# SciML/NonlinearSolve.jl

Hardware: AMD Instinct MI355X
Metric: newton_steps_per_sec (higher is better)
Workload: dtype f64; 1 GPU; bratu2d_1024x1024_newtonraphson_gmres30_fixedwork_csr_spmv; unknowns_global=1048576, unknowns_per_gpu=1048576, arnoldi_steps_per_newton_step=30, ortho=sstep_auto_auto, parallelism=row-range x1, comm=none

## Files before the change

include/mi355x_nk.h:

```cpp
#ifndef MI355X_NK_H
#define MI355X_NK_H

#include <stdint.h>
#include <stddef.h>

#ifdef __cplusplus
extern "C" {
#endif

#define NK_VERSION_MAJOR 0
#define NK_VERSION_MINOR 1

typedef enum {
  NK_OK = 0,
  NK_E_INVALID = -1,
  NK_E_HIP = -2,
  NK_E_RCCL = -3,
  NK_E_NOMEM = -4,
  NK_E_UNSUPPORTED = -5,
  NK_E_CALLBACK = -6,
  NK_E_SINGULAR = -7,
  NK_E_COMM = -8
} nk_status;

// ... 194 lines not shown
int nk_ctx_comm_init_callbacks(nk_ctx *ctx, int nranks, int rank, const nk_comm_callbacks *cb);
#define NK_IPC_HANDLE_BYTES 64
int nk_ctx_comm_peer_handle(nk_ctx *ctx, int64_t arena_bytes, char handle_out[NK_IPC_HANDLE_BYTES]);
int nk_ctx_comm_enable_peer(nk_ctx *ctx, const char *handles);
int nk_ctx_comm_peer_status(nk_ctx *ctx, int *enabled, int64_t *errors);
int nk_ctx_comm_allreduce(nk_ctx *ctx, double *buf, int count, int op);
int nk_ctx_comm_peer_selftest(nk_ctx *ctx, int *ok);
int nk_ctx_comm_peer_disable(nk_ctx *ctx);
int nk_ctx_comm_info(nk_ctx *ctx, int *kind, int *nranks, int *rank);
int nk_ctx_comm_device_shared(nk_ctx *ctx, int *shared);

int nk_partition_range(int64_t n_global, int64_t granule, int nranks, int rank,
                       int64_t *row_begin, int64_t *row_end);

int nk_csr_create(nk_ctx *ctx, int64_t nrows_local, int64_t n_global, int64_t row_begin, int64_t nnz,
                  int index_bits, int index_base, const void *rowptr, const void *colind,
                  const double *vals, int memspace, nk_csr **out);
int nk_csr_create_from_csc(nk_ctx *ctx, int64_t n, int64_t nnz, int index_bits, int index_base,
                           const void *colptr, const void *rowval, const double *nzval, nk_csr **out);
int nk_csr_create_from_csc_rows(nk_ctx *ctx, int64_t n, int64_t nnz, int index_bits, int index_base,
                                const void *colptr, const void *rowval, const double *nzval,
                                int64_t row_begin, int64_t nrows_local, nk_csr **out);
int nk_csr_destroy(nk_csr *A);
int nk_csr_set_values(nk_csr *A, const double *vals, int memspace);
int nk_csr_set_values_csc(nk_csr *A, const double *nzval, int64_t nnz_csc, int memspace);
int nk_csr_get_values(nk_csr *A, double *vals, int memspace);
int nk_csr_info(nk_csr *A, int64_t *nrows_local, int64_t *n_global, int64_t *nnz, int64_t *n_halo);
double *nk_csr_values_device(nk_csr *A);
int nk_spmv(nk_csr *A, const double *x, double *y, int memspace);
int nk_spmv_t(nk_csr *A, const double *x, double *y, int memspace);
int nk_csr_powers(nk_csr *A, const double *x, double *Y, int64_t ldy, int s, const double *theta, double scale, int memspace,
                  int *resident);
int nk_csr_powers_layout(int64_t nrows, const int32_t *rowptr, const int32_t *col, int num_cus, int layout[6]);
int nk_csr_colsumsq(nk_csr *A, double *out, int memspace);

int nk_problem_create(nk_ctx *ctx, int kind, const double *params, int nparams, nk_problem **out);
int nk_problem_create_user(nk_ctx *ctx, int64_t n_local, int64_t n_global, int64_t row_begin,
                           const nk_user_callbacks *cb, void *user, nk_csr *jac_pattern,
                           nk_problem **out);
int nk_problem_destroy(nk_problem *P);
int nk_problem_size(nk_problem *P, int64_t *n_local, int64_t *n_global, int64_t *row_begin);
int nk_problem_set_params(nk_problem *P, const double *params, int nparams);
int nk_problem_initial_guess(nk_problem *P, double *u0, int memspace);
int nk_residual(nk_problem *P, const double *u, double *f, int memspace);
int nk_jvp(nk_problem *P, const double *u, const double *v, double *Jv, int memspace);
int nk_vjp(nk_problem *P, const double *u, const double *v, double *vJ, int memspace);
int nk_problem_jac_csr(nk_problem *P, nk_csr **out);
int nk_jac_values(nk_problem *P, const double *u, int memspace, nk_csr *J);
int nk_jac_values_colored(nk_problem *P, const double *u, int memspace, nk_csr *J, int *ncolors);

int nk_gmres_create(nk_ctx *ctx, int64_t n_local, int restart_m, int ortho, nk_gmres **out);
int nk_gmres_destroy(nk_gmres *G);
int nk_gmres_set_operator_csr(nk_gmres *G, nk_csr *A);
int nk_gmres_set_operator_jvp(nk_gmres *G, nk_problem *P, const double *u, int memspace);
int nk_gmres_set_operator_fn(nk_gmres *G, nk_matvec_fn fn, void *user);
int nk_gmres_set_normal_form(nk_gmres *G, int on);
int nk_gmres_set_block_size(nk_gmres *G, int s);
int nk_gmres_set_sstep_basis(nk_gmres *G, int basis);
int nk_gmres_set_spectrum_interval(nk_gmres *G, double lo, double hi);
int nk_gmres_get_sstep_state(nk_gmres *G, int *block_size, int *newton_basis, int *breakdowns);
int nk_gmres_set_normal_form_damping(nk_gmres *G, const double *d_diag, double lambda);
int nk_gmres_set_shift(nk_gmres *G, double sigma);
int nk_gmres_set_shift_weights(nk_gmres *G, const double *d_m);
int nk_gmres_set_right_preconditioner(nk_gmres *G, nk_matvec_fn fn, void *user);
int nk_gmres_set_left_preconditioner(nk_gmres *G, nk_matvec_fn fn, void *user);
int nk_gmres_set_left_preconditioner_host(nk_gmres *G, nk_matvec_fn fn, void *user);
// ... 118 lines not shown
```

nonlinearsolve.jl_amd/_lib.py:

```python
from __future__ import annotations

import ctypes as C
import os
import subprocess

_HERE = os.path.dirname(os.path.abspath(__file__))
LIB_PATH = os.environ.get("NK_LIB_PATH") or os.path.join(_HERE, "lib", "libmi355x_nk.so")
CSRC = os.path.join(_HERE, "csrc")


class NKError(RuntimeError):
    pass


HOST, DEVICE = 0, 1
BATCH_ANALYTIC_JAC, BATCH_FLOAT32 = 1, 2
RET_NAMES = ["Default", "Success", "MaxIters", "Unstable", "Stalled", "InternalLinearSolveFailed",
             "ShrinkThresholdExceeded", "MaxTime", "Failure", "InternalLineSearchFailed"]
PROBLEM_QUADRATIC, PROBLEM_BRATU2D, PROBLEM_BRUSSELATOR2D, PROBLEM_USER = 1, 2, 3, 100
ALG_NEWTON_RAPHSON, ALG_TRUST_REGION, ALG_GAUSS_NEWTON, ALG_LEVENBERG_MARQUARDT, ALG_PSEUDO_TRANSIENT = 0, 1, 2, 3, 4
LINSOLVE_GMRES_MATFREE, LINSOLVE_GMRES_CSR, LINSOLVE_BANDED_LU = 0, 1, 2
ORTHO_MGS, ORTHO_CGS2, ORTHO_CGS, ORTHO_DCGS2, ORTHO_DCGS2_1R, ORTHO_SSTEP = 0, 1, 2, 3, 4, 5
FORCING_NONE, FORCING_EW2 = 0, 1
COMM_NONE, COMM_RCCL, COMM_CALLBACKS = 0, 1, 2
# ... 86 lines not shown
    "nk_ctx_synchronize": (_I, [_P]),
    "nk_ctx_set_halo_overlap": (_I, [_P, _I]),
    "nk_ctx_set_deterministic": (_I, [_P, _I]),
    "nk_ctx_profile_enable": (_I, [_P, _I]),
    "nk_ctx_profile_kernel_count": (_I, []),
    "nk_ctx_profile_query": (_I, [_P, _I, C.POINTER(C.c_char_p), C.POINTER(_L), C.POINTER(_D), C.POINTER(_D)]),
    "nk_comm_unique_id": (_I, [C.c_char_p]),
    "nk_ctx_comm_init_rccl": (_I, [_P, _I, _I, C.c_char_p]),
    "nk_ctx_comm_init_callbacks": (_I, [_P, _I, _I, C.POINTER(CommCallbacks)]),
    "nk_ctx_comm_info": (_I, [_P, C.POINTER(_I), C.POINTER(_I), C.POINTER(_I)]),
    "nk_ctx_comm_device_shared": (_I, [_P, C.POINTER(_I)]),
    "nk_ctx_comm_peer_handle": (_I, [_P, _L, C.c_char_p]),
    "nk_ctx_comm_enable_peer": (_I, [_P, C.c_char_p]),
    "nk_ctx_comm_peer_status": (_I, [_P, C.POINTER(_I), C.POINTER(_L)]),
    "nk_ctx_comm_peer_selftest": (_I, [_P, C.POINTER(_I)]),
    "nk_ctx_comm_peer_disable": (_I, [_P]),
    "nk_ctx_comm_allreduce": (_I, [_P, _P, _I, _I]),
    "nk_vec_axpby": (_I, [_P, _L, _D, _P, _D, _P]),
    "nk_vec_fill": (_I, [_P, _L, _D, _P]),
    "nk_partition_range": (_I, [_L, _L, _I, _I, C.POINTER(_L), C.POINTER(_L)]),
    "nk_csr_create": (_I, [_P, _L, _L, _L, _L, _I, _I, _P, _P, _P, _I, _PP]),
    "nk_csr_create_from_csc": (_I, [_P, _L, _L, _I, _I, _P, _P, _P, _PP]),
    "nk_csr_create_from_csc_rows": (_I, [_P, _L, _L, _I, _I, _P, _P, _P, _L, _L, _PP]),
    "nk_csr_destroy": (_I, [_P]),
    "nk_csr_set_values": (_I, [_P, _P, _I]),
    "nk_csr_get_values": (_I, [_P, _P, _I]),
    "nk_csr_set_values_csc": (_I, [_P, _P, _L, _I]),
    "nk_csr_info": (_I, [_P, C.POINTER(_L), C.POINTER(_L), C.POINTER(_L), C.POINTER(_L)]),
    "nk_csr_values_device": (_P, [_P]),
    "nk_spmv": (_I, [_P, _P, _P, _I]),
    "nk_spmv_t": (_I, [_P, _P, _P, _I]),
    "nk_csr_powers": (_I, [_P, _P, _P, _L, _I, _P, _D, _I, _P]),
    "nk_csr_powers_layout": (_I, [_L, _P, _P, _I, _P]),
    "nk_csr_colsumsq": (_I, [_P, _P, _I]),
    "nk_gmres_set_normal_form_damping": (_I, [_P, _P, C.c_double]),
    "nk_gmres_set_shift": (_I, [_P, C.c_double]),
    "nk_gmres_set_block_size": (_I, [_P, _I]),
    "nk_gmres_set_sstep_basis": (_I, [_P, _I]),
    "nk_gmres_set_spectrum_interval": (_I, [_P, C.c_double, C.c_double]),
    "nk_gmres_get_sstep_state": (_I, [_P, C.POINTER(_I), C.POINTER(_I), C.POINTER(_I)]),
    "nk_gmres_set_shift_weights": (_I, [_P, _P]),
    "nk_problem_create": (_I, [_P, _I, C.POINTER(_D), _I, _PP]),
    "nk_problem_create_user": (_I, [_P, _L, _L, _L, C.POINTER(UserCallbacks), _P, _P, _PP]),
    "nk_problem_destroy": (_I, [_P]),
    "nk_problem_size": (_I, [_P, C.POINTER(_L), C.POINTER(_L), C.POINTER(_L)]),
    "nk_problem_set_params": (_I, [_P, C.POINTER(_D), _I]),
    "nk_problem_initial_guess": (_I, [_P, _P, _I]),
    "nk_residual": (_I, [_P, _P, _P, _I]),
    "nk_jvp": (_I, [_P, _P, _P, _P, _I]),
    "nk_vjp": (_I, [_P, _P, _P, _P, _I]),
    "nk_problem_jac_csr": (_I, [_P, _PP]),
    "nk_jac_values": (_I, [_P, _P, _I, _P]),
    "nk_jac_values_colored": (_I, [_P, _P, _I, _P, C.POINTER(_I)]),
    "nk_gmres_create": (_I, [_P, _L, _I, _I, _PP]),
    "nk_gmres_destroy": (_I, [_P]),
    "nk_gmres_set_operator_csr": (_I, [_P, _P]),
    "nk_gmres_set_operator_jvp": (_I, [_P, _P, _P, _I]),
    "nk_gmres_set_operator_fn": (_I, [_P, MATVEC_FN, _P]),
    "nk_gmres_set_normal_form": (_I, [_P, _I]),
    "nk_gmres_set_right_preconditioner": (_I, [_P, MATVEC_FN, _P]),
    "nk_gmres_set_operator_fn_host": (_I, [_P, MATVEC_FN, _P]),
    "nk_gmres_set_right_preconditioner_host": (_I, [_P, MATVEC_FN, _P]),
    "nk_gmres_set_left_preconditioner": (_I, [_P, MATVEC_FN, _P]),
    "nk_gmres_set_left_preconditioner_host": (_I, [_P, MATVEC_FN, _P]),
    "nk_gmres_set_preconditioner": (_I, [_P, _I, _P]),
    "nk_precond_create_jacobi": (_I, [_P, _PP]),
# ... 98 lines not shown
```

nonlinearsolve.jl_amd/core.py:

```python
from __future__ import annotations

import ctypes as C
from dataclasses import dataclass, field
from typing import Callable, Optional, Sequence

import numpy as np

from . import _lib as L
from ._lib import NKError, check

try:
    import torch
except Exception:
    torch = None


def _is_torch(x):
    return torch is not None and isinstance(x, torch.Tensor)


def _ptr(x, n: Optional[int] = None):
    if _is_torch(x):
        if x.dtype != torch.float64:
            raise TypeError("device vectors must be float64")
# ... 252 lines not shown
        p, ms, _k = _ptr(vals, self.info()["nnz"])
        check(L.lib().nk_csr_set_values(self._h, p, ms))

    def values(self):
        out = np.empty(self.info()["nnz"])
        check(L.lib().nk_csr_get_values(self._h, C.c_void_p(out.ctypes.data), L.HOST))
        return out

    def values_device(self):
        return _view(L.lib().nk_csr_values_device(self._h), self.info()["nnz"])

    def matvec(self, x, out=None):
        n = self.info()["nrows_local"]
        px, ms, _k = _ptr(x, n)
        y = _like(x, n) if out is None else out
        py, ms2, _k2 = _ptr(y, n)
        if ms != ms2:
            raise ValueError("x and out must live in the same memory space")
        check(L.lib().nk_spmv(self._h, px, py, ms))
        return y

    def powers(self, x, s, theta=None, scale=1.0):
        n = self.info()["nrows_local"]
        px, ms, _k = _ptr(x, n)
        Y = _like(x, n * s)
        pY, _ms2, _k2 = _ptr(Y, n * s)
        th = None if theta is None else np.ascontiguousarray(theta, dtype=np.float64)
        if th is not None and th.size != s:
            raise ValueError("theta must have s entries")
        res = C.c_int(0)
        check(L.lib().nk_csr_powers(self._h, px, pY, n, int(s), None if th is None else C.c_void_p(th.ctypes.data),
                                    float(scale), ms, C.byref(res)))
        return Y.reshape(s, n), bool(res.value)

    @staticmethod
    def powers_layout(A, num_cus: int = 256):
        import numpy as _np
        A = A.tocsr()
        rp = _np.ascontiguousarray(A.indptr, dtype=_np.int32)
        ci = _np.ascontiguousarray(A.indices, dtype=_np.int32)
        out = (C.c_int * 6)()
        check(L.lib().nk_csr_powers_layout(int(A.shape[0]), C.c_void_p(rp.ctypes.data), C.c_void_p(ci.ctypes.data), int(num_cus), out))
        return {"kind": ("none", "bands", "segments")[out[0]], "slices": out[1], "slots": out[2], "bands": out[3],
                "segments": out[4], "ring": bool(out[5])}

    def rmatvec(self, x, out=None):
        n = self.info()["nrows_local"]
        px, ms, _k = _ptr(x, n)
        y = _like(x, n) if out is None else out
        py, _ms2, _k2 = _ptr(y, n)
        check(L.lib().nk_spmv_t(self._h, px, py, ms))
        return y

    def colsumsq(self, like=None):
        n = self.info()["nrows_local"]
        y = np.empty(n) if like is None else _like(like, n)
        py, ms, _k = _ptr(y, n)
        check(L.lib().nk_csr_colsumsq(self._h, py, ms))
        return y

    __matmul__ = matvec

    def close(self):
        if self._h and self._owned:
            L.lib().nk_csr_destroy(self._h)
        self._h = None
# ... 1209 lines not shown
```

nonlinearsolve.jl_amd/csrc/nk_powers.hip:

```cpp
#include <algorithm>
#include <stdlib.h>
#include <vector>

#include "nk_internal.h"

constexpr int PW_T = 1024;
constexpr int PW_HALO = 1024;
constexpr int PW_FLAG_STRIDE = 16;
constexpr int PW_NXCD = 8;

struct pw_args {
  int nrows, nb, s, variant;
  const int32_t *rowptr, *col;
  const double *val;
  const double *x0;
  double *Y;
  int64_t ldy;
  const double *scal_first, *scal_rest, *theta;
  const int *d_skip;
  uint64_t *flags;
  uint64_t base;
  uint64_t *err;
  int ns;
  double c_lap;
  const double *diag;
  int seg_len, ring;
  struct {
    int up, dn;
    const int32_t *halo_vl;
    double *push_up, *push_dn;
    uint64_t *flag_up, *flag_dn;
    const double *recv_up, *recv_dn;
    const uint64_t *myflag_up, *myflag_dn;
    uint64_t *err;
    int ebuf;
  } pr;
};

constexpr int PW_NST = 12, PW_STP = 16;
__device__ unsigned long long *g_pw_stamp = nullptr;
#ifdef NK_PW_STAMPS
#define PW_STAMP(p, i) do { if (t == 0 && (p) < PW_STP) s_pw_st[(p) * PW_NST + (i)] = wall_clock64(); } while (0)
#else
#define PW_STAMP(p, i) do { } while (0)
#endif

__device__ __forceinline__ int pw_band_of(int bid, int nb) {
  const int q = nb / PW_NXCD, r = nb % PW_NXCD;
  const int x = bid % PW_NXCD, k = bid / PW_NXCD;
  return x * q + (x < r ? x : r) + k;
}
__device__ __forceinline__ void pw_store_sc1(double *p, double v) {
  __hip_atomic_store(reinterpret_cast<unsigned long long *>(p), (unsigned long long)__double_as_longlong(v), __ATOMIC_RELAXED,
                     __HIP_MEMORY_SCOPE_AGENT);
}
// ... 15 lines not shown
      }
    }
  }
}
__device__ __forceinline__ bool pw_wait_peer(const uint64_t *f, uint64_t target, uint64_t *perr, uint64_t *err) {
  if (__hip_atomic_load(f, __ATOMIC_ACQUIRE, __HIP_MEMORY_SCOPE_SYSTEM) >= target) return true;
  const unsigned long long t0 = wall_clock64(), lim = nk_peer_timeout(perr);
  for (unsigned it = 1;; ++it) {
    __builtin_amdgcn_s_sleep(1);
    if (__hip_atomic_load(f, __ATOMIC_ACQUIRE, __HIP_MEMORY_SCOPE_SYSTEM) >= target) return true;
    if ((it & 63u) == 0) {
      if (__hip_atomic_load(err, __ATOMIC_RELAXED, __HIP_MEMORY_SCOPE_SYSTEM) != 0) return false;
      if (__hip_atomic_load(perr, __ATOMIC_RELAXED, __HIP_MEMORY_SCOPE_AGENT) > 4 || wall_clock64() - t0 > lim) {
        atomicAdd((unsigned long long *)perr, 1ull);
        __hip_atomic_store(err, (uint64_t)1, __ATOMIC_RELAXED, __HIP_MEMORY_SCOPE_SYSTEM);
        return false;
      }
    }
  }
}
__device__ __forceinline__ void pw_store_sys(double *p, double v) {
  __hip_atomic_store(reinterpret_cast<unsigned long long *>(p), (unsigned long long)__double_as_longlong(v), __ATOMIC_RELAXED,
                     __HIP_MEMORY_SCOPE_SYSTEM);
}
__device__ __forceinline__ double pw_load_sys(const double *p) {
  return __longlong_as_double((long long)__hip_atomic_load(reinterpret_cast<const unsigned long long *>(p), __ATOMIC_RELAXED,
                                                           __HIP_MEMORY_SCOPE_SYSTEM));
}
template <int RPT>
__device__ __forceinline__ constexpr int pw_slice(int q) {
  return q == 0 ? 0 : (q == 1 ? RPT - 1 : q - 1);
}

template <int RPT, int W, int GEN, bool PEER = false>
__global__ __launch_bounds__(PW_T) void k_spmv_powers(const pw_args a) {
  if (a.d_skip != nullptr && *a.d_skip != 0) return;
  extern __shared__ double pw_x[];
  __shared__ int s_abort;
#ifdef NK_PW_STAMPS
  __shared__ unsigned long long s_pw_st[PW_STP * PW_NST];
  for (int i = threadIdx.x; i < PW_STP * PW_NST; i += PW_T) s_pw_st[i] = 0;
#endif
  constexpr int RB = PW_T * RPT, XN = RB + 2 * PW_HALO;
  constexpr int NBND = RPT > 1 ? 2 : 1;
  const int t = threadIdx.x;
  const int b = pw_band_of(blockIdx.x, a.nb);
  const int r0 = b * RB;
  double *xa = pw_x, *xb = pw_x + XN;
  const bool pup = PEER && b == 0 && a.pr.up != 0, pdn = PEER && b == a.nb - 1 && a.pr.dn != 0;

  double v[RPT][W];
  int ci[RPT][W];
  int len[RPT];
  if constexpr (GEN == 1) {
    static_assert(W >= 5, "the 5-point stencil needs five slots per row");
#pragma unroll
    for (int i = 0; i < RPT; ++i) {
      const int r = r0 + t + PW_T * i;
      const int rc = r < a.nrows ? r : a.nrows - 1;
      const int gj = rc / a.ns, gi = rc - gj * a.ns;
      const double dd = a.diag[rc];
      const int base = rc - (r0 - PW_HALO), own = PW_HALO + t + PW_T * i;
      const bool hs = gj > 0, hw = gi > 0, he = gi + 1 < a.ns, hn = gj + 1 < a.ns;
      const int pW = hs ? 1 : 0, pC = pW + (hw ? 1 : 0), pE = pC + 1, pN = pE + (he ? 1 : 0), n = pN + (hn ? 1 : 0);
      const double off = -a.c_lap, ctr = 4.0 * a.c_lap - dd;
#pragma unroll
      for (int j = 0; j < W; ++j) {
        double vv = 0.0;
        int cc = own;
        if (hs && j == 0) { vv = off; cc = base - a.ns; }
        if (hw && j == pW) { vv = off; cc = base - 1; }
        if (j == pC) { vv = ctr; cc = base; }
        if (he && j == pE) { vv = off; cc = base + 1; }
        if (hn && j == pN) { vv = off; cc = base + a.ns; }
        v[i][j] = vv;
        ci[i][j] = cc;
      }
      len[i] = r < a.nrows ? n : 0;
    }
  } else if constexpr (W > 8) {
#pragma unroll
    for (int i = 0; i < RPT; ++i) {
      const int r = r0 + t + PW_T * i;
      const int rc = r < a.nrows ? r : a.nrows - 1;
      const int k0 = a.rowptr[rc], k1 = a.rowptr[rc + 1];
      len[i] = r < a.nrows ? k1 - k0 : 0;
#pragma unroll
// ... 11 lines not shown
    for (int i = 0; i < RPT; ++i) {
      const int rfirst = r0 + PW_T * i;
      const int r = rfirst + t;
      const int rc = r < a.nrows ? r : a.nrows - 1;
      const int k0 = a.rowptr[rc], k1 = a.rowptr[rc + 1];
      const int rl = rfirst < a.nrows ? (rfirst + PW_T <= a.nrows ? rfirst + PW_T : a.nrows) : rfirst;
      const int kb = rfirst < a.nrows ? a.rowptr[rfirst] : 0, ke = rfirst < a.nrows ? a.rowptr[rl] : 0;
      len[i] = r < a.nrows ? k1 - k0 : 0;
#pragma unroll
      for (int j = 0; j < W; ++j) {
        const int e = t + PW_T * j;
        if (kb + e < ke) { sv[e] = a.val[kb + e]; sc[e] = a.col[kb + e]; }
      }
      __syncthreads();
#pragma unroll
      for (int j = 0; j < W; ++j) {
        const int e = (j < len[i]) ? k0 - kb + j : 0;
        const double vv = sv[e];
        int c = sc[e];
        if (PEER && (pup || pdn) && j < len[i] && c >= a.nrows) c = a.pr.halo_vl[c - a.nrows];
        v[i][j] = (j < len[i]) ? vv : 0.0;
        ci[i][j] = (j < len[i]) ? c - (r0 - PW_HALO) : PW_HALO + t + PW_T * i;
      }
      __syncthreads();
    }
  }
  for (int idx = t; idx < XN; idx += PW_T) {
    const int g = r0 - PW_HALO + idx;
    xa[idx] = (g >= 0 && g < a.nrows) ? a.x0[g] : 0.0;
    xb[idx] = 0.0;
  }
  if (t == 0) s_abort = 0;
  __syncthreads();
  if (PEER && (pup || pdn)) {
    if (pup) pw_store_sys(a.pr.push_up + (size_t)a.pr.ebuf * PW_T + t, a.x0[t]);
    if (pdn) pw_store_sys(a.pr.push_dn + (size_t)a.pr.ebuf * PW_T + t, a.x0[a.nrows - PW_T + t]);
    __threadfence_system();
    __syncthreads();
    if (t == 0 && pup) __hip_atomic_store(a.pr.flag_up, a.base, __ATOMIC_RELEASE, __HIP_MEMORY_SCOPE_SYSTEM);
    if (t == 64 && pdn) __hip_atomic_store(a.pr.flag_dn, a.base, __ATOMIC_RELEASE, __HIP_MEMORY_SCOPE_SYSTEM);
    if (t == 0 && pup && !pw_wait_peer(a.pr.myflag_up, a.base, a.pr.err, a.err)) s_abort = 1;
    if (t == 64 && pdn && !pw_wait_peer(a.pr.myflag_dn, a.base, a.pr.err, a.err)) s_abort = 1;
    __syncthreads();
    if (s_abort) return;
    if (pup) xa[t] = pw_load_sys(a.pr.recv_up + (size_t)a.pr.ebuf * PW_T + t);
    if (pdn) xa[PW_HALO + RB + t] = pw_load_sys(a.pr.recv_dn + (size_t)a.pr.ebuf * PW_T + t);
    __syncthreads();
  }

  const bool shifted = a.theta != nullptr;
  for (int p = 0; p < a.s; ++p) {
    const double *xin = (p & 1) ? xb : xa;
    double *xout = (p & 1) ? xa : xb;
    const double *osp = (p == 0) ? a.scal_first : a.scal_rest;
    const double os = osp ? *osp : 1.0;
    const double th = shifted ? a.theta[p] : 0.0;
    double *ycol = a.Y + (int64_t)p * a.ldy;
    const bool pub = p + 1 < a.s;
    PW_STAMP(p, 0);
#pragma unroll
    for (int q = 0; q < RPT; ++q) {
      const int i = pw_slice<RPT>(q);
      const int lr = t + PW_T * i, r = r0 + lr;
      double sum = 0.0;
#pragma unroll
      for (int j = 0; j < W; ++j) {
        const double pr = v[i][j] * xin[ci[i][j]];
        sum = (j < len[i]) ? sum + pr : sum;
      }
      double out = shifted ? sum - th * xin[PW_HALO + lr] : sum;
      out = osp ? os * out : out;
      if (r < a.nrows) {
        xout[PW_HALO + lr] = out;
        if (q < NBND) pw_store_sc1(ycol + r, out);
        else ycol[r] = out;
      }
      if (PEER && pub) {
        const size_t boff = (size_t)(a.pr.ebuf + ((p + 1) & 1)) * PW_T + t;
        if (pup && i == 0) pw_store_sys(a.pr.push_up + boff, out);
        if (pdn && i == RPT - 1) pw_store_sys(a.pr.push_dn + boff, out);
      }
      if (q == NBND - 1) PW_STAMP(p, 1);
      if (pub && (a.variant & 255) == 0 && q == NBND - 1) {
        if (PEER && (pup || pdn)) __threadfence_system();
        asm volatile("s_waitcnt vmcnt(0)" ::: "memory");
        PW_STAMP(p, 2);
        __syncthreads();
        PW_STAMP(p, 3);
        if (t == 0 && !((a.variant & 256) && b == 0))
          __hip_atomic_store(a.flags + (size_t)b * PW_FLAG_STRIDE, a.base + (uint64_t)p + 1, __ATOMIC_RELAXED,
                             __HIP_MEMORY_SCOPE_AGENT);
        if (PEER) {
          if (t == 64 && pup) __hip_atomic_store(a.pr.flag_up, a.base + (uint64_t)p + 1, __ATOMIC_RELEASE, __HIP_MEMORY_SCOPE_SYSTEM);
          if (t == 128 && pdn) __hip_atomic_store(a.pr.flag_dn, a.base + (uint64_t)p + 1, __ATOMIC_RELEASE, __HIP_MEMORY_SCOPE_SYSTEM);
        }
      }
    }
    PW_STAMP(p, 4);
    if (!pub) break;
    if ((a.variant & 255) != 0) {
      if (PEER && (pup || pdn)) __threadfence_system();
      asm volatile("s_waitcnt vmcnt(0)" ::: "memory");
      __syncthreads();
      if (t == 0)
        __hip_atomic_store(a.flags + (size_t)b * PW_FLAG_STRIDE, a.base + (uint64_t)p + 1, __ATOMIC_RELAXED,
                           __HIP_MEMORY_SCOPE_AGENT);
      if (PEER) {
        if (t == 64 && pup) __hip_atomic_store(a.pr.flag_up, a.base + (uint64_t)p + 1, __ATOMIC_RELEASE, __HIP_MEMORY_SCOPE_SYSTEM);
        if (t == 128 && pdn) __hip_atomic_store(a.pr.flag_dn, a.base + (uint64_t)p + 1, __ATOMIC_RELEASE, __HIP_MEMORY_SCOPE_SYSTEM);
      }
    }
    if (t == 0) {
      if (b > 0) {
        if (!pw_wait(a.flags + (size_t)(b - 1) * PW_FLAG_STRIDE, a.base + (uint64_t)p + 1, a.err)) s_abort = 1;
      } else if (PEER && pup) {
        if (!pw_wait_peer(a.pr.myflag_up, a.base + (uint64_t)p + 1, a.pr.err, a.err)) s_abort = 1;
      }
    }
    PW_STAMP(p, 5);
    if (t == 64) {
      if (b + 1 < a.nb) {
        if (!pw_wait(a.flags + (size_t)(b + 1) * PW_FLAG_STRIDE, a.base + (uint64_t)p + 1, a.err)) s_abort = 1;
      } else if (PEER && pdn) {
        if (!pw_wait_peer(a.pr.myflag_dn, a.base + (uint64_t)p + 1, a.pr.err, a.err)) s_abort = 1;
      }
    }
    __syncthreads();
    PW_STAMP(p, 6);
    if (s_abort) return;
    {
      const int gu = r0 - PW_HALO + t, gd = r0 + RB + t;
// ... 113 lines not shown
    __syncthreads();
    if (t == 0 && !((a.variant & 256) && b == 0))
      __hip_atomic_store(a.flags + (size_t)b * PW_FLAG_STRIDE, a.base + (uint64_t)p + 1, __ATOMIC_RELAXED, __HIP_MEMORY_SCOPE_AGENT);
    if (t == 0 && nup >= 0) {
      if (!pw_wait(a.flags + (size_t)nup * PW_FLAG_STRIDE, a.base + (uint64_t)p + 1, a.err)) s_abort = 1;
    }
    if (t == 64 && ndn >= 0) {
      if (!pw_wait(a.flags + (size_t)ndn * PW_FLAG_STRIDE, a.base + (uint64_t)p + 1, a.err)) s_abort = 1;
    }
    __syncthreads();
    if (s_abort) return;
    {
      double hu[SEG], hd[SEG];
      int lu = b0 - PW_HALO + t, ld = b0 + RB + t;
      if (ring) { lu = lu < 0 ? lu + M : lu; ld = ld >= M ? ld - M : ld; }
#pragma unroll
      for (int sg = 0; sg < SEG; ++sg) {
        hu[sg] = (nup >= 0 && lu >= 0 && lu < M) ? pw_load_sc1(ycol + sg * M + lu) : 0.0;
        hd[sg] = (ndn >= 0 && ld < M) ? pw_load_sc1(ycol + sg * M + ld) : 0.0;
      }
#pragma unroll
      for (int sg = 0; sg < SEG; ++sg) {
        xout[sg * XS + t] = hu[sg];
        xout[sg * XS + PW_HALO + RB + t] = hd[sg];
      }
    }
    __syncthreads();
  }
}

struct nk_powers_plan {
  int rpt = 0, w = 0, nb = 0;
  int seg = 0, ring = 0, seg_len = 0;
  uint64_t *d_flags = nullptr;
  uint64_t *h_err = nullptr, *h_err_dev = nullptr;
  uint64_t epoch = 0;
  bool broken = false;
  int strikes = 0;
  bool peer = false;
  nk_peer_powers pp;
  int32_t *d_halo_vl = nullptr;
};
void nk_powers_plan_destroy(nk_powers_plan *P) {
  if (!P) return;
  hipFree(P->d_flags);
  hipFree(P->d_halo_vl);
  if (P->h_err) hipHostFree(P->h_err);
  delete P;
}
static int pw_variant() {
  static const int v = getenv("NK_PW_VARIANT") ? atoi(getenv("NK_PW_VARIANT")) : 0;
  static const std::vector<long> stalls = [] {
    std::vector<long> v;
    const char *e = getenv("NK_PW_DEBUG_STALL_LAUNCH");
    while (e && *e) {
      char *end = nullptr;
      const long x = strtol(e, &end, 10);
      if (end == e) break;
      v.push_back(x);
      e = (*end == ',') ? end + 1 : end;
    }
    return v;
  }();
  static long launches = 0;
  ++launches;
  bool stall = false;
  for (long x : stalls) stall = stall || (x > 0 && launches == x);
  return (v & 255) | (stall ? 256 : 0);
}
static bool pw_enabled() {
  static const bool on = !(getenv("NK_SPMV_POWERS") && atoi(getenv("NK_SPMV_POWERS")) == 0);
  return on;
}

template <int RPT, int W, int GEN, bool PEER = false>
static int pw_launch(nk_ctx *ctx, const pw_args &a, bool query, int *occ) {
  constexpr size_t lds_x = (size_t)2 * (PW_T * RPT + 2 * PW_HALO) * sizeof(double), lds_m = (W > 8 || GEN == 1) ? 0 : (size_t)PW_T * W * 12;
  constexpr size_t lds = lds_x > lds_m ? lds_x : lds_m;
  if (lds > 64 * 1024)
    NK_HIP(hipFuncSetAttribute(reinterpret_cast<const void *>(&k_spmv_powers<RPT, W, GEN, PEER>),
                               hipFuncAttributeMaxDynamicSharedMemorySize, (int)lds));
  if (query) {
    NK_HIP(hipOccupancyMaxActiveBlocksPerMultiprocessor(occ, k_spmv_powers<RPT, W, GEN, PEER>, PW_T, lds));
    return NK_OK;
  }
  hipEvent_t e0 = nullptr, e1 = nullptr;
  static const bool coop = getenv("NK_PW_COOP") && atoi(getenv("NK_PW_COOP")) != 0;
  if (ctx->prof.on && nk_prof_next(ctx, &e0, &e1))
    hipExtLaunchKernelGGL((k_spmv_powers<RPT, W, GEN, PEER>), dim3(a.nb), dim3(PW_T), lds, ctx->stream, e0, e1, 0, a);
  else if (coop) {
    pw_args ac = a;
    void *args[] = {(void *)&ac};
    NK_HIP(hipLaunchCooperativeKernel(reinterpret_cast<const void *>(&k_spmv_powers<RPT, W, GEN, PEER>), dim3(a.nb), dim3(PW_T), args,
                                      (unsigned int)lds, ctx->stream));
  } else
    hipLaunchKernelGGL((k_spmv_powers<RPT, W, GEN, PEER>), dim3(a.nb), dim3(PW_T), lds, ctx->stream, a);
  NK_HIP(hipGetLastError());
  return NK_OK;
}
static int pw_dispatch(nk_ctx *ctx, int rpt, int w, const pw_args &a, bool query, int *occ, int gen = 0, bool peer = false) {
  if (peer) {
#define PW_PEER(R, WW) if (rpt == R && w == WW) return pw_launch<R, WW, 0, true>(ctx, a, query, occ)
    PW_PEER(1, 5); PW_PEER(2, 5); PW_PEER(4, 5); PW_PEER(6, 5);
    PW_PEER(1, 8); PW_PEER(2, 8);
    PW_PEER(1, 16);
#undef PW_PEER
    NK_FAIL(NK_E_INVALID, "internal: no matrix-powers kernel for %d rows per thread × %d entries per row", rpt, w);
  }
#define PW_CASE(R, WW, G) if (rpt == R && w == WW && gen == G) return pw_launch<R, WW, G>(ctx, a, query, occ)
  PW_CASE(1, 5, 1); PW_CASE(2, 5, 1); PW_CASE(4, 5, 1); PW_CASE(6, 5, 1);
  PW_CASE(1, 5, 0); PW_CASE(2, 5, 0); PW_CASE(4, 5, 0); PW_CASE(6, 5, 0);
  PW_CASE(1, 8, 0); PW_CASE(2, 8, 0);
  PW_CASE(1, 16, 0);
#undef PW_CASE
  NK_FAIL(NK_E_INVALID, "internal: no matrix-powers kernel for %d rows per thread × %d entries per row", rpt, w);
}

template <int RPS, int W, int SEG>
static int pw_launch_seg(nk_ctx *ctx, const pw_args &a, bool query, int *occ) {
  constexpr size_t lds_x = (size_t)2 * SEG * (PW_T * RPS + 2 * PW_HALO) * sizeof(double), lds_m = (size_t)PW_T * W * 12;
  constexpr size_t lds = lds_x > lds_m ? lds_x : lds_m;
  if (lds > 64 * 1024)
    NK_HIP(hipFuncSetAttribute(reinterpret_cast<const void *>(&k_spmv_powers_seg<RPS, W, SEG>), hipFuncAttributeMaxDynamicSharedMemorySize,
                               (int)lds));
  if (query) {
    NK_HIP(hipOccupancyMaxActiveBlocksPerMultiprocessor(occ, k_spmv_powers_seg<RPS, W, SEG>, PW_T, lds));
    return NK_OK;
  }
  hipEvent_t e0 = nullptr, e1 = nullptr;
  if (ctx->prof.on && nk_prof_next(ctx, &e0, &e1))
    hipExtLaunchKernelGGL((k_spmv_powers_seg<RPS, W, SEG>), dim3(a.nb), dim3(PW_T), lds, ctx->stream, e0, e1, 0, a);
  else
    hipLaunchKernelGGL((k_spmv_powers_seg<RPS, W, SEG>), dim3(a.nb), dim3(PW_T), lds, ctx->stream, a);
  NK_HIP(hipGetLastError());
  return NK_OK;
}
static bool pw_seg_shape(int rps, int w, int seg) {
  if (seg == 1) return (w == 5 && (rps == 1 || rps == 2 || rps == 4)) || (w == 8 && (rps == 1 || rps == 2));
  if (seg == 2) return (w == 5 && (rps == 1 || rps == 2)) || (w == 8 && rps == 1);
  return false;
}
static int pw_dispatch_seg(nk_ctx *ctx, int rps, int w, int seg, const pw_args &a, bool query, int *occ) {
#define PW_SEG(R, WW, SG) if (rps == R && w == WW && seg == SG) return pw_launch_seg<R, WW, SG>(ctx, a, query, occ)
  PW_SEG(1, 5, 1); PW_SEG(2, 5, 1); PW_SEG(4, 5, 1); PW_SEG(1, 8, 1); PW_SEG(2, 8, 1);
  PW_SEG(1, 5, 2); PW_SEG(2, 5, 2); PW_SEG(1, 8, 2);
#undef PW_SEG
  NK_FAIL(NK_E_INVALID, "internal: no segmented matrix-powers kernel for %d slices × %d slots × %d segments", rps, w, seg);
// ... 41 lines not shown
      for (int64_t r = 0; r < n && ok; ++r) {
        const int64_t b0 = (r / rb) * rb, lo = b0 - PW_HALO, hi = b0 + rb + PW_HALO;
        for (int32_t k = rowptr[r]; k < rowptr[r + 1]; ++k)
          if (col[k] < lo || col[k] >= hi) { ok = false; break; }
      }
      if (!ok) continue;
      L.kind = 1; L.rpt = rpt; L.w = w; L.nb = (int)((n + rb - 1) / rb); L.seg = 1; L.ring = 0; L.M = n;
      return L;
    }
    const int seg = lay == 1 ? 1 : 2, ring = lay == 2 ? 0 : 1;
    if (n % seg) continue;
    const int64_t M = n / seg, pc = (M + num_cus - 1) / num_cus;
    const int nd = (int)((pc + PW_T - 1) / PW_T);
    const int rps = nd <= 1 ? 1 : (nd <= 2 ? 2 : (nd <= 4 ? 4 : 0));
    if (!rps || !pw_seg_shape(rps, w, seg)) continue;
    const int64_t RB = (int64_t)PW_T * rps;
    if (ring && (M % RB)) continue;
    bool ok = true;
    for (int64_t r = 0; r < n && ok; ++r) {
      const int64_t b0 = ((r % M) / RB) * RB;
      for (int32_t k = rowptr[r]; k < rowptr[r + 1]; ++k) {
        if (col[k] < 0 || col[k] >= n) { ok = false; break; }
        int64_t d = (int64_t)col[k] % M - b0;
        if (ring) d = d < -PW_HALO ? d + M : (d >= RB + PW_HALO ? d - M : d);
        if (d < -PW_HALO || d >= RB + PW_HALO) { ok = false; break; }
      }
    }
    if (!ok) continue;
    L.kind = 2; L.rpt = rps; L.w = w; L.nb = (int)((M + RB - 1) / RB); L.seg = seg; L.ring = ring; L.M = M;
    return L;
  }
  return L;
}
static int pw_layout_index(const pw_layout &L) { return L.kind == 1 ? 0 : (L.seg == 1 ? 1 : (L.ring ? 3 : 2)); }
extern "C" int nk_csr_powers_layout(int64_t nrows, const int32_t *rowptr, const int32_t *col, int num_cus, int layout[6]) {
  NK_REQUIRE(rowptr && col && layout && nrows >= 0 && num_cus >= 1, "bad argument");
  const pw_layout L = pw_find_layout(nrows, rowptr, col, num_cus, 0);
  layout[0] = L.kind; layout[1] = L.rpt; layout[2] = L.w; layout[3] = L.nb; layout[4] = L.seg; layout[5] = L.ring;
  return NK_OK;
}

static int pw_plan_ranks(nk_csr *A) {
  nk_ctx *ctx = A->ctx;
  const int64_t n = A->nrows;
  const int nh = (int)A->halo_gcols.size();
  std::vector<int32_t> hvl(nh > 0 ? nh : 1, 0), vcol;
  bool ok = pw_enabled() && ctx->peer.on && !ctx->device_shared && n >= PW_T && A->nnz >= 1;
  static const bool ranks_off = getenv("NK_PW_RANKS") && atoi(getenv("NK_PW_RANKS")) == 0;
  ok = ok && !ranks_off;
  for (int h = 0; h < nh && ok; ++h) {
    const int64_t vl = A->halo_gcols[h] - A->row_begin;
    ok = (vl < 0 && vl >= -PW_HALO && ctx->rank > 0) || (vl >= n && vl < n + PW_HALO && ctx->rank + 1 < ctx->nranks);
    hvl[h] = (int32_t)vl;
  }
  pw_layout L;
  if (ok) {
    vcol.resize(A->h_col.size());
    for (size_t k = 0; k < vcol.size(); ++k) vcol[k] = A->h_col[k] < n ? A->h_col[k] : hvl[A->h_col[k] - n];
    L = pw_find_layout(n, A->h_rowptr.data(), vcol.data(), ctx->num_cus, 0);
    ok = L.kind == 1 && n % ((int64_t)PW_T * L.rpt) == 0;
    if (ok) {
      pw_args probe{};
      int occ = 0;
      NK_TRY(pw_dispatch(ctx, L.rpt, L.w, probe, true, &occ, 0, true));
      ok = occ >= 1 && L.nb <= ctx->num_cus * occ;
    }
  }
  nk_peer_powers pp;
  bool all = false;
  NK_TRY(nk_peer_powers_setup(ctx, ok, &pp, &all));
  if (!all) return NK_OK;
  NK_TRY(pw_plan_new(A->ctx, L.rpt, L.w, L.nb, &A->pw));
  A->pw->peer = true;
  A->pw->pp = pp;
  NK_HIP(hipMalloc((void **)&A->pw->d_halo_vl, hvl.size() * sizeof(int32_t)));
  NK_HIP(nk_memcpy(ctx, A->pw->d_halo_vl, hvl.data(), hvl.size() * sizeof(int32_t), hipMemcpyHostToDevice));
  return NK_OK;
}
static int pw_plan(nk_csr *A) {
  if (A->pw_tried) return NK_OK;
  A->pw_tried = true;
  nk_ctx *ctx = A->ctx;
  if (ctx->nranks > 1 && A->local_only) return NK_OK;
  if (ctx->nranks > 1) return pw_plan_ranks(A);
  if (!pw_enabled() || !A->halo_gcols.empty() || A->nrows < 1 || A->nnz < 1) return NK_OK;
  pw_args probe{};
  for (int skip = 0; skip < 4;) {
    const pw_layout L = pw_find_layout(A->nrows, A->h_rowptr.data(), A->h_col.data(), ctx->num_cus, skip);
    if (!L.kind) return NK_OK;
    int occ = 0;
    if (L.kind == 1) NK_TRY(pw_dispatch(ctx, L.rpt, L.w, probe, true, &occ));
    else NK_TRY(pw_dispatch_seg(ctx, L.rpt, L.w, L.seg, probe, true, &occ));
    if (occ >= 1 && L.nb <= ctx->num_cus * occ) {
      NK_TRY(pw_plan_new(A->ctx, L.rpt, L.w, L.nb, &A->pw));
      if (L.kind == 2) { A->pw->seg = L.seg; A->pw->ring = L.ring; A->pw->seg_len = (int)L.M; }
      return NK_OK;
    }
    skip = pw_layout_index(L) + 1;
  }
  return NK_OK;
}
bool nk_csr_powers_ready(nk_csr *A) {
  if (!A->pw_tried && pw_plan(A) != NK_OK) return false;
  return A->pw != nullptr && !A->pw->broken && A->pw->h_err[0] == 0;
}
int nk_csr_powers_check(nk_csr *A) {
  if (!A->pw || A->pw->broken || A->pw->h_err[0] == 0) return NK_OK;
  A->pw->broken = true;
  A->pw->strikes++;
  NK_FAIL(NK_E_HIP, "resident matrix-powers kernel: a workgroup waited longer than NK_PW_TIMEOUT_MS for its neighbour band "
                    "(NK_SPMV_POWERS=0 keeps the streaming SpMV)");
}
static void pw_rearm(nk_powers_plan *P) {
  if (!P || !P->broken || P->peer || P->strikes >= 3) return;
  P->h_err[0] = 0;
  P->broken = false;
}
void nk_csr_powers_rearm(nk_csr *A) { if (A) pw_rearm(A->pw); }
void nk_problem_powers_rearm(nk_problem *P) { if (P) pw_rearm(P->pw); }
int nk_csr_powers_dev(nk_csr *A, const double *d_x0, double *d_Y, int64_t ldy, int s, const double *d_scal_first,
                      const double *d_scal_rest, const double *d_theta, const int *d_skip) {
  NK_REQUIRE(nk_csr_powers_ready(A), "internal: matrix powers on a matrix without a plan");
  NK_REQUIRE(s >= 1 && s <= 200, "matrix powers: 1 ≤ s ≤ 200");
  nk_ctx *ctx = A->ctx;
  nk_powers_plan *P = A->pw;
  pw_args a{};
  a.nrows = (int)A->nrows; a.nb = P->nb; a.s = s; a.variant = pw_variant();
  a.rowptr = A->d_rowptr; a.col = A->d_col; a.val = A->d_val;
  a.x0 = d_x0; a.Y = d_Y; a.ldy = ldy;
  a.scal_first = d_scal_first; a.scal_rest = d_scal_rest; a.theta = d_theta; a.d_skip = d_skip;
  a.flags = P->d_flags; a.base = (++P->epoch) << 8; a.err = P->h_err_dev;
  ctx->stats.op_applies += s;
  nk_prof_scope prof_(ctx, NK_K_POWERS,
                      (double)s * (12.0 * (double)A->nnz + 4.0 * (double)(A->nrows + 1) + 16.0 * (double)A->nrows));
  if (P->seg > 0) {
    a.seg_len = P->seg_len; a.ring = P->ring;
    return pw_dispatch_seg(ctx, P->rpt, P->w, P->seg, a, false, nullptr);
  }
  if (P->peer) {
    a.pr.up = ctx->rank > 0; a.pr.dn = ctx->rank + 1 < ctx->nranks;
    a.pr.halo_vl = P->d_halo_vl;
    a.pr.push_up = P->pp.push_up; a.pr.push_dn = P->pp.push_dn; a.pr.flag_up = P->pp.flag_up; a.pr.flag_dn = P->pp.flag_dn;
    a.pr.recv_up = P->pp.recv_up; a.pr.recv_dn = P->pp.recv_dn; a.pr.myflag_up = P->pp.myflag_up; a.pr.myflag_dn = P->pp.myflag_dn;
    a.pr.err = nk_peer_err_ptr(ctx);
    a.pr.ebuf = (int)(P->epoch & 1) * 2;
    ctx->stats.halo_exchanges++;
    return pw_dispatch(ctx, P->rpt, P->w, a, false, nullptr, 0, true);
  }
  return pw_dispatch(ctx, P->rpt, P->w, a, false, nullptr);
}

static int pw_problem_plan(nk_problem *P) {
  if (P->pw_tried) return NK_OK;
  P->pw_tried = true;
  nk_ctx *ctx = P->ctx;
  if (!pw_enabled() || P->kind != NK_PROBLEM_BRATU2D || ctx->nranks != 1 || P->replicated || P->j0 != 0 || P->j1 != P->ns ||
      P->ns < 2 || P->ns > PW_HALO || P->n_local != P->ns * P->ns)
    return NK_OK;
  const int64_t n = P->n_local, per_cu = (n + ctx->num_cus - 1) / ctx->num_cus;
  const int need = (int)((per_cu + PW_T - 1) / PW_T);
  const int rpt = need <= 1 ? 1 : (need <= 2 ? 2 : (need <= 4 ? 4 : (need <= 6 ? 6 : 0)));
  if (!rpt) return NK_OK;
  const int nb = (int)((n + (int64_t)PW_T * rpt - 1) / ((int64_t)PW_T * rpt));
  pw_args probe{};
  int occ = 0;
  NK_TRY(pw_dispatch(ctx, rpt, 5, probe, true, &occ, 1));
  if (occ < 1 || nb > ctx->num_cus * occ) return NK_OK;
  return pw_plan_new(P->ctx, rpt, 5, nb, &P->pw);
}
bool nk_problem_powers_ready(nk_problem *P) {
  if (!P->pw_tried && pw_problem_plan(P) != NK_OK) return false;
// ... 92 lines not shown
```

Baseline: 2432 newton_steps/s.

## Add stencil-offset form for resident matrix-powers kernel with per-row presence masks

When every block of rows has at most W distinct column offsets, the planner now builds a per-block offset table and a per-row bitmask of which offsets are present. The kernel then replaces per-entry column indices with those offsets, which removes the column-index loads and the indirect gather. For the 5-point pattern it also takes the centre, north and south neighbours from registers instead of LDS. This costs host-side analysis at plan time, extra template instantiations and one more LDS staging pass for the values. The path is on by default and can be turned off with NK_PW_OFFSETS=0.

```diff
diff --git a/include/mi355x_nk.h b/include/mi355x_nk.h
--- a/include/mi355x_nk.h
+++ b/include/mi355x_nk.h
@@ -250,6 +250,11 @@
 int nk_csr_powers(nk_csr *A, const double *x, double *Y, int64_t ldy, int s, const double *theta, double scale, int memspace,
                   int *resident);
 int nk_csr_powers_layout(int64_t nrows, const int32_t *rowptr, const int32_t *col, int num_cus, int layout[6]);
+#define NK_PW_FORM_NONE 0
+#define NK_PW_FORM_BANDS 1
+#define NK_PW_FORM_SEGMENTS 2
+#define NK_PW_FORM_OFFSETS 3
+int nk_csr_powers_form(nk_csr *A, int *form);
 int nk_csr_colsumsq(nk_csr *A, double *out, int memspace);
 
 int nk_problem_create(nk_ctx *ctx, int kind, const double *params, int nparams, nk_problem **out);
diff --git a/nonlinearsolve.jl_amd/_lib.py b/nonlinearsolve.jl_amd/_lib.py
--- a/nonlinearsolve.jl_amd/_lib.py
+++ b/nonlinearsolve.jl_amd/_lib.py
@@ -142,6 +142,7 @@
     "nk_spmv_t": (_I, [_P, _P, _P, _I]),
     "nk_csr_powers": (_I, [_P, _P, _P, _L, _I, _P, _D, _I, _P]),
     "nk_csr_powers_layout": (_I, [_L, _P, _P, _I, _P]),
+    "nk_csr_powers_form": (_I, [_P, _P]),
     "nk_csr_colsumsq": (_I, [_P, _P, _I]),
     "nk_gmres_set_normal_form_damping": (_I, [_P, _P, C.c_double]),
     "nk_gmres_set_shift": (_I, [_P, C.c_double]),
diff --git a/nonlinearsolve.jl_amd/core.py b/nonlinearsolve.jl_amd/core.py
--- a/nonlinearsolve.jl_amd/core.py
+++ b/nonlinearsolve.jl_amd/core.py
@@ -308,6 +308,11 @@
         check(L.lib().nk_csr_powers(self._h, px, pY, n, int(s), None if th is None else C.c_void_p(th.ctypes.data),
                                     float(scale), ms, C.byref(res)))
         return Y.reshape(s, n), bool(res.value)
+
+    def powers_form(self):
+        f = C.c_int(0)
+        check(L.lib().nk_csr_powers_form(self._h, C.byref(f)))
+        return ("none", "bands", "segments", "offsets")[f.value]
 
     @staticmethod
     def powers_layout(A, num_cus: int = 256):
diff --git a/nonlinearsolve.jl_amd/csrc/nk_powers.hip b/nonlinearsolve.jl_amd/csrc/nk_powers.hip
--- a/nonlinearsolve.jl_amd/csrc/nk_powers.hip
+++ b/nonlinearsolve.jl_amd/csrc/nk_powers.hip
@@ -21,6 +21,8 @@
   uint64_t *flags;
   uint64_t base;
   uint64_t *err;
+  const int32_t *offs;
+  const uint8_t *pmask;
   int ns;
   double c_lap;
   const double *diag;
@@ -102,7 +104,13 @@
   return q == 0 ? 0 : (q == 1 ? RPT - 1 : q - 1);
 }
 
-template <int RPT, int W, int GEN, bool PEER = false>
+constexpr int PW_K_LDS = 0, PW_K_C = 1, PW_K_N = 2, PW_K_S = 3;
+constexpr int pw_ks(int k0, int k1, int k2, int k3, int k4) { return k0 | k1 << 2 | k2 << 4 | k3 << 6 | k4 << 8; }
+constexpr int PW_KS_5PT_1024 = pw_ks(PW_K_S, PW_K_LDS, PW_K_C, PW_K_LDS, PW_K_N);
+constexpr int PW_KS_CENTRE2 = pw_ks(PW_K_LDS, PW_K_LDS, PW_K_C, PW_K_LDS, PW_K_LDS);
+constexpr int PW_KS_LDS = 0;
+
+template <int RPT, int W, int GEN, bool PEER = false, int KS = 0>
 __global__ __launch_bounds__(PW_T) void k_spmv_powers(const pw_args a) {
   if (a.d_skip != nullptr && *a.d_skip != 0) return;
   extern __shared__ double pw_x[];
@@ -122,7 +130,38 @@
   double v[RPT][W];
   int ci[RPT][W];
   int len[RPT];
-  if constexpr (GEN == 1) {
+  int o[W];
+  unsigned pm[RPT];
+  double xr[RPT];
+  if constexpr (GEN == 2) {
+    double *sv = pw_x;
+#pragma unroll
+    for (int j = 0; j < W; ++j) o[j] = a.offs[b * W + j];
+#pragma unroll
+    for (int i = 0; i < RPT; ++i) {
+      const int rfirst = r0 + PW_T * i;
+      const int r = rfirst + t;
+      const int rc = r < a.nrows ? r : a.nrows - 1;
+      const int k0 = a.rowptr[rc];
+      const int rl = rfirst < a.nrows ? (rfirst + PW_T <= a.nrows ? rfirst + PW_T : a.nrows) : rfirst;
+      const int kb = rfirst < a.nrows ? a.rowptr[rfirst] : 0, ke = rfirst < a.nrows ? a.rowptr[rl] : 0;
+      pm[i] = r < a.nrows ? (unsigned)a.pmask[rc] : 0u;
+#pragma unroll
+      for (int j = 0; j < W; ++j) {
+        const int e = t + PW_T * j;
+        if (kb + e < ke) sv[e] = a.val[kb + e];
+      }
+      __syncthreads();
+      int k = k0 - kb;
+#pragma unroll
+      for (int j = 0; j < W; ++j) {
+        const bool h = (pm[i] >> j) & 1u;
+        v[i][j] = h ? sv[h ? k : 0] : 0.0;
+        k += h ? 1 : 0;
+      }
+      __syncthreads();
+    }
+  } else if constexpr (GEN == 1) {
     static_assert(W >= 5, "the 5-point stencil needs five slots per row");
 #pragma unroll
     for (int i = 0; i < RPT; ++i) {
@@ -200,6 +239,10 @@
   }
   if (t == 0) s_abort = 0;
   __syncthreads();
+  if constexpr (GEN == 2) {
+#pragma unroll
+    for (int i = 0; i < RPT; ++i) xr[i] = xa[PW_HALO + t + PW_T * i];
+  }
   if (PEER && (pup || pdn)) {
     if (pup) pw_store_sys(a.pr.push_up + (size_t)a.pr.ebuf * PW_T + t, a.x0[t]);
     if (pdn) pw_store_sys(a.pr.push_dn + (size_t)a.pr.ebuf * PW_T + t, a.x0[a.nrows - PW_T + t]);
@@ -230,13 +273,29 @@
     for (int q = 0; q < RPT; ++q) {
       const int i = pw_slice<RPT>(q);
       const int lr = t + PW_T * i, r = r0 + lr;
-      double sum = 0.0;
-#pragma unroll
-      for (int j = 0; j < W; ++j) {
-        const double pr = v[i][j] * xin[ci[i][j]];
-        sum = (j < len[i]) ? sum + pr : sum;
-      }
-      double out = shifted ? sum - th * xin[PW_HALO + lr] : sum;
+      double sum = 0.0, out;
+      if constexpr (GEN == 2) {
+        const double *xl = xin + PW_HALO + lr;
+        const double xc = xr[i], xn = xr[i + 1 < RPT ? i + 1 : i], xs = xr[i > 0 ? i - 1 : i];
+#pragma unroll
+        for (int j = 0; j < W; ++j) {
+          const int kd = (KS >> (2 * j)) & 3;
+          double xv;
+          if (kd == PW_K_C) xv = xc;
+          else if (kd == PW_K_N && i + 1 < RPT) xv = xn;
+          else if (kd == PW_K_S && i > 0) xv = xs;
+          else xv = xl[o[j]];
+          if ((pm[i] >> j) & 1u) sum = sum + v[i][j] * xv;
+        }
+        out = shifted ? sum - th * xr[i] : sum;
+      } else {
+#pragma unroll
+        for (int j = 0; j < W; ++j) {
+          const double pr = v[i][j] * xin[ci[i][j]];
+          sum = (j < len[i]) ? sum + pr : sum;
+        }
+        out = shifted ? sum - th * xin[PW_HALO + lr] : sum;
+      }
       out = osp ? os * out : out;
       if (r < a.nrows) {
         xout[PW_HALO + lr] = out;
@@ -265,6 +324,10 @@
       }
     }
     PW_STAMP(p, 4);
+    if constexpr (GEN == 2) {
+#pragma unroll
+      for (int i = 0; i < RPT; ++i) xr[i] = xout[PW_HALO + t + PW_T * i];
+    }
     if (!pub) break;
     if ((a.variant & 255) != 0) {
       if (PEER && (pup || pdn)) __threadfence_system();
@@ -444,6 +507,10 @@
 struct nk_powers_plan {
   int rpt = 0, w = 0, nb = 0;
   int seg = 0, ring = 0, seg_len = 0;
+  int form = 0;
+  int ks = 0;
+  int32_t *d_offs = nullptr;
+  uint8_t *d_pmask = nullptr;
   uint64_t *d_flags = nullptr;
   uint64_t *h_err = nullptr, *h_err_dev = nullptr;
   uint64_t epoch = 0;
@@ -457,6 +524,8 @@
   if (!P) return;
   hipFree(P->d_flags);
   hipFree(P->d_halo_vl);
+  hipFree(P->d_offs);
+  hipFree(P->d_pmask);
   if (P->h_err) hipHostFree(P->h_err);
   delete P;
 }
@@ -480,37 +549,42 @@
   for (long x : stalls) stall = stall || (x > 0 && launches == x);
   return (v & 255) | (stall ? 256 : 0);
 }
+static bool pw_offsets_enabled() {
+  static const bool on = !(getenv("NK_PW_OFFSETS") && atoi(getenv("NK_PW_OFFSETS")) == 0);
+  return on;
+}
 static bool pw_enabled() {
   static const bool on = !(getenv("NK_SPMV_POWERS") && atoi(getenv("NK_SPMV_POWERS")) == 0);
   return on;
 }
 
-template <int RPT, int W, int GEN, bool PEER = false>
+template <int RPT, int W, int GEN, bool PEER = false, int KS = 0>
 static int pw_launch(nk_ctx *ctx, const pw_args &a, bool query, int *occ) {
-  constexpr size_t lds_x = (size_t)2 * (PW_T * RPT + 2 * PW_HALO) * sizeof(double), lds_m = (W > 8 || GEN == 1) ? 0 : (size_t)PW_T * W * 12;
+  constexpr size_t lds_x = (size_t)2 * (PW_T * RPT + 2 * PW_HALO) * sizeof(double), lds_m = (W > 8 || GEN == 1) ? 0 : (size_t)PW_T * W * (GEN == 2 ? 8 : 12);
   constexpr size_t lds = lds_x > lds_m ? lds_x : lds_m;
   if (lds > 64 * 1024)
-    NK_HIP(hipFuncSetAttribute(reinterpret_cast<const void *>(&k_spmv_powers<RPT, W, GEN, PEER>),
+    NK_HIP(hipFuncSetAttribute(reinterpret_cast<const void *>(&k_spmv_powers<RPT, W, GEN, PEER, KS>),
                                hipFuncAttributeMaxDynamicSharedMemorySize, (int)lds));
   if (query) {
-    NK_HIP(hipOccupancyMaxActiveBlocksPerMultiprocessor(occ, k_spmv_powers<RPT, W, GEN, PEER>, PW_T, lds));
+    NK_HIP(hipOccupancyMaxActiveBlocksPerMultiprocessor(occ, k_spmv_powers<RPT, W, GEN, PEER, KS>, PW_T, lds));
     return NK_OK;
   }
   hipEvent_t e0 = nullptr, e1 = nullptr;
   static const bool coop = getenv("NK_PW_COOP") && atoi(getenv("NK_PW_COOP")) != 0;
   if (ctx->prof.on && nk_prof_next(ctx, &e0, &e1))
-    hipExtLaunchKernelGGL((k_spmv_powers<RPT, W, GEN, PEER>), dim3(a.nb), dim3(PW_T), lds, ctx->stream, e0, e1, 0, a);
+    hipExtLaunchKernelGGL((k_spmv_powers<RPT, W, GEN, PEER, KS>), dim3(a.nb), dim3(PW_T), lds, ctx->stream, e0, e1, 0, a);
   else if (coop) {
     pw_args ac = a;
     void *args[] = {(void *)&ac};
-    NK_HIP(hipLaunchCooperativeKernel(reinterpret_cast<const void *>(&k_spmv_powers<RPT, W, GEN, PEER>), dim3(a.nb), dim3(PW_T), args,
+    NK_HIP(hipLaunchCooperativeKernel(reinterpret_cast<const void *>(&k_spmv_powers<RPT, W, GEN, PEER, KS>), dim3(a.nb), dim3(PW_T), args,
                                       (unsigned int)lds, ctx->stream));
   } else
-    hipLaunchKernelGGL((k_spmv_powers<RPT, W, GEN, PEER>), dim3(a.nb), dim3(PW_T), lds, ctx->stream, a);
+    hipLaunchKernelGGL((k_spmv_powers<RPT, W, GEN, PEER, KS>), dim3(a.nb), dim3(PW_T), lds, ctx->stream, a);
   NK_HIP(hipGetLastError());
   return NK_OK;
 }
-static int pw_dispatch(nk_ctx *ctx, int rpt, int w, const pw_args &a, bool query, int *occ, int gen = 0, bool peer = false) {
+static int pw_dispatch(nk_ctx *ctx, int rpt, int w, const pw_args &a, bool query, int *occ, int gen = 0, bool peer = false,
+                       int ks = 0) {
   if (peer) {
 #define PW_PEER(R, WW) if (rpt == R && w == WW) return pw_launch<R, WW, 0, true>(ctx, a, query, occ)
     PW_PEER(1, 5); PW_PEER(2, 5); PW_PEER(4, 5); PW_PEER(6, 5);
@@ -525,6 +599,15 @@
   PW_CASE(1, 8, 0); PW_CASE(2, 8, 0);
   PW_CASE(1, 16, 0);
 #undef PW_CASE
+  if (gen == 2) {
+#define PW_OFS(R, WW, K) if (rpt == R && w == WW && ks == K) return pw_launch<R, WW, 2, false, K>(ctx, a, query, occ)
+    PW_OFS(1, 5, PW_KS_LDS); PW_OFS(2, 5, PW_KS_LDS); PW_OFS(4, 5, PW_KS_LDS); PW_OFS(6, 5, PW_KS_LDS);
+    PW_OFS(1, 5, PW_KS_CENTRE2); PW_OFS(2, 5, PW_KS_CENTRE2); PW_OFS(4, 5, PW_KS_CENTRE2); PW_OFS(6, 5, PW_KS_CENTRE2);
+    PW_OFS(2, 5, PW_KS_5PT_1024); PW_OFS(4, 5, PW_KS_5PT_1024); PW_OFS(6, 5, PW_KS_5PT_1024);
+    PW_OFS(1, 8, PW_KS_LDS); PW_OFS(2, 8, PW_KS_LDS);
+#undef PW_OFS
+    NK_FAIL(NK_E_INVALID, "internal: no stencil-offset matrix-powers kernel for %d rows per thread × %d slots, kinds %d", rpt, w, ks);
+  }
   NK_FAIL(NK_E_INVALID, "internal: no matrix-powers kernel for %d rows per thread × %d entries per row", rpt, w);
 }
 
@@ -632,6 +715,49 @@
   }
   return L;
 }
+static bool pw_find_offsets(int64_t n, const int32_t *rowptr, const int32_t *col, int rpt, int w, int nb, std::vector<int32_t> &offs,
+                            std::vector<uint8_t> &mask) {
+  if (w > 8) return false;
+  const int64_t rb = (int64_t)PW_T * rpt;
+  offs.assign((size_t)nb * w, 0);
+  mask.assign((size_t)n, 0);
+  for (int b = 0; b < nb; ++b) {
+    const int64_t lo = (int64_t)b * rb, hi = std::min(n, lo + rb);
+    int32_t set[8];
+    int ns = 0;
+    for (int64_t r = lo; r < hi; ++r)
+      for (int32_t k = rowptr[r]; k < rowptr[r + 1]; ++k) {
+        if (k > rowptr[r] && col[k] <= col[k - 1]) return false;
+        const int64_t d = (int64_t)col[k] - r;
+        if (d < -PW_HALO || d > PW_HALO) return false;
+        const int pos = (int)(std::lower_bound(set, set + ns, (int32_t)d) - set);
+        if (pos < ns && set[pos] == d) continue;
+        if (ns == w) return false;
+        std::copy_backward(set + pos, set + ns, set + ns + 1);
+        set[pos] = (int32_t)d;
+        ++ns;
+      }
+    std::copy(set, set + ns, offs.begin() + (size_t)b * w);
+    for (int64_t r = lo; r < hi; ++r)
+      for (int32_t k = rowptr[r]; k < rowptr[r + 1]; ++k)
+        mask[r] |= (uint8_t)(1u << (std::lower_bound(set, set + ns, (int32_t)(col[k] - r)) - set));
+  }
+  return true;
+}
+static int pw_offsets_ks(const std::vector<int32_t> &offs, int rpt, int w) {
+  const int cand[3] = {PW_KS_5PT_1024, PW_KS_CENTRE2, PW_KS_LDS};
+  for (int ks : cand) {
+    if (w != 5 && ks != PW_KS_LDS) continue;
+    if (rpt == 1 && ks == PW_KS_5PT_1024) continue;
+    bool ok = true;
+    for (size_t k = 0; k < offs.size() && ok; ++k) {
+      const int kd = (ks >> (2 * (int)(k % w))) & 3;
+      ok = (kd == PW_K_LDS) || (kd == PW_K_C && offs[k] == 0) || (kd == PW_K_N && offs[k] == PW_T) || (kd == PW_K_S && offs[k] == -PW_T);
+    }
+    if (ok) return ks;
+  }
+  return PW_KS_LDS;
+}
 static int pw_layout_index(const pw_layout &L) { return L.kind == 1 ? 0 : (L.seg == 1 ? 1 : (L.ring ? 3 : 2)); }
 extern "C" int nk_csr_powers_layout(int64_t nrows, const int32_t *rowptr, const int32_t *col, int num_cus, int layout[6]) {
   NK_REQUIRE(rowptr && col && layout && nrows >= 0 && num_cus >= 1, "bad argument");
@@ -672,6 +798,7 @@
   if (!all) return NK_OK;
   NK_TRY(pw_plan_new(A->ctx, L.rpt, L.w, L.nb, &A->pw));
   A->pw->peer = true;
+  A->pw->form = NK_PW_FORM_BANDS;
   A->pw->pp = pp;
   NK_HIP(hipMalloc((void **)&A->pw->d_halo_vl, hvl.size() * sizeof(int32_t)));
   NK_HIP(nk_memcpy(ctx, A->pw->d_halo_vl, hvl.data(), hvl.size() * sizeof(int32_t), hipMemcpyHostToDevice));
@@ -693,7 +820,25 @@
     else NK_TRY(pw_dispatch_seg(ctx, L.rpt, L.w, L.seg, probe, true, &occ));
     if (occ >= 1 && L.nb <= ctx->num_cus * occ) {
       NK_TRY(pw_plan_new(A->ctx, L.rpt, L.w, L.nb, &A->pw));
-      if (L.kind == 2) { A->pw->seg = L.seg; A->pw->ring = L.ring; A->pw->seg_len = (int)L.M; }
+      nk_powers_plan *Q = A->pw;
+      Q->form = L.kind == 1 ? NK_PW_FORM_BANDS : NK_PW_FORM_SEGMENTS;
+      if (L.kind == 2) { Q->seg = L.seg; Q->ring = L.ring; Q->seg_len = (int)L.M; }
+      std::vector<int32_t> offs;
+      std::vector<uint8_t> mask;
+      if (L.kind == 1 && pw_offsets_enabled() &&
+          pw_find_offsets(A->nrows, A->h_rowptr.data(), A->h_col.data(), L.rpt, L.w, L.nb, offs, mask)) {
+        int occ2 = 0;
+        const int ks = pw_offsets_ks(offs, L.rpt, L.w);
+        NK_TRY(pw_dispatch(ctx, L.rpt, L.w, probe, true, &occ2, 2, false, ks));
+        if (occ2 >= 1 && L.nb <= ctx->num_cus * occ2) {
+          NK_HIP(hipMalloc((void **)&Q->d_offs, offs.size() * sizeof(int32_t)));
+          NK_HIP(hipMalloc((void **)&Q->d_pmask, mask.size()));
+          NK_HIP(nk_memcpy(ctx, Q->d_offs, offs.data(), offs.size() * sizeof(int32_t), hipMemcpyHostToDevice));
+          NK_HIP(nk_memcpy(ctx, Q->d_pmask, mask.data(), mask.size(), hipMemcpyHostToDevice));
+          Q->form = NK_PW_FORM_OFFSETS;
+          Q->ks = ks;
+        }
+      }
       return NK_OK;
     }
     skip = pw_layout_index(L) + 1;
@@ -703,6 +848,12 @@
 bool nk_csr_powers_ready(nk_csr *A) {
   if (!A->pw_tried && pw_plan(A) != NK_OK) return false;
   return A->pw != nullptr && !A->pw->broken && A->pw->h_err[0] == 0;
+}
+extern "C" int nk_csr_powers_form(nk_csr *A, int *form) {
+  NK_REQUIRE(A && form, "bad argument");
+  NK_HIP(hipSetDevice(A->ctx->device));
+  *form = nk_csr_powers_ready(A) ? A->pw->form : NK_PW_FORM_NONE;
+  return NK_OK;
 }
 int nk_csr_powers_check(nk_csr *A) {
   if (!A->pw || A->pw->broken || A->pw->h_err[0] == 0) return NK_OK;
@@ -737,6 +888,10 @@
     a.seg_len = P->seg_len; a.ring = P->ring;
     return pw_dispatch_seg(ctx, P->rpt, P->w, P->seg, a, false, nullptr);
   }
+  if (P->form == NK_PW_FORM_OFFSETS) {
+    a.offs = P->d_offs; a.pmask = P->d_pmask;
+    return pw_dispatch(ctx, P->rpt, P->w, a, false, nullptr, 2, false, P->ks);
+  }
   if (P->peer) {
     a.pr.up = ctx->rank > 0; a.pr.dn = ctx->rank + 1 < ctx->nranks;
     a.pr.halo_vl = P->d_halo_vl;
```

Measured after the change: 2430 newton_steps/s (median of 4 runs). About the same (-0.1%).
